# ZenHKD/ocr-vi-invoice

Measured on AMD Instinct MI355X. Metric: invoice images/sec end-to-end (det+rec), higher is better.
Workload: dtype f16x2

## Files before the change

### ocr_vi_invoice_amd/csrc/attention.hip

```cpp
#include <stdlib.h>

#include "kernels.h"

namespace ocrvi {
OCRVI_RANGE_FLAG_TU()


template <typename T> struct AttnCfg;
template <> struct AttnCfg<float> {
    static constexpr int KROW = 128;
    static constexpr __host__ __device__ int vstride(int NP) { return NP * 4 + 16; }
};
template <> struct AttnCfg<bf16_t> {
    static constexpr int KROW = 64;
    static constexpr __host__ __device__ int vstride(int NP) { return (NP * 2 + 255) / 256 * 256 + 16; }
};
template <> struct AttnCfg<f16_t> : AttnCfg<bf16_t> {};
template <> struct AttnCfg<f16x2_t> : AttnCfg<float> {};

__device__ __forceinline__ int swz64(int row) { return (-(row >> 2)) & 3; }

template <typename T> __device__ __forceinline__ f32x4 mfma16(const uint4& a, const uint4& b, f32x4 c);
template <> __device__ __forceinline__ f32x4 mfma16<bf16_t>(const uint4& a, const uint4& b, f32x4 c) {
    return __builtin_amdgcn_mfma_f32_16x16x32_bf16(__builtin_bit_cast(bf16x8, a), __builtin_bit_cast(bf16x8, b), c, 0, 0, 0);
}
template <> __device__ __forceinline__ f32x4 mfma16<f16_t>(const uint4& a, const uint4& b, f32x4 c) {
    return __builtin_amdgcn_mfma_f32_16x16x32_f16(__builtin_bit_cast(f16x8, a), __builtin_bit_cast(f16x8, b), c, 0, 0, 0);
}

__device__ __forceinline__ void split_pair(float a, float b, unsigned& H, unsigned& L) {
    typedef float f2v __attribute__((ext_vector_type(2)));
    typedef _Float16 h2v __attribute__((ext_vector_type(2)));
    H = __builtin_bit_cast(unsigned, __builtin_convertvector((f2v){a, b}, h2v));
    const float la = fma_mix_lo(-1.0f, H, a), lb = fma_mix_hi(-1.0f, H, b);
    L = __builtin_bit_cast(unsigned, __builtin_convertvector((f2v){la, lb}, h2v));
}

template <typename T, int MAXT, bool MASK, int NWV = 4>
__global__ __launch_bounds__(NWV * 64, (IsSplit<T>::value && MAXT <= 16 && NWV == 8) ? 4 : 1) void attention_kernel(const T* __restrict__ qkv, T* __restrict__ out, int N, int heads, int kbase, int Nk,
                                                                                                               float* __restrict__ po, float2* __restrict__ pml) {
    constexpr int EPC = TypeInfo<T>::EPC;
    constexpr int KROW = AttnCfg<T>::KROW;
    constexpr int CH = KROW / 16;
    extern __shared__ __attribute__((aligned(16))) char smem[];
    const int L = xcd_remap(blockIdx.x, gridDim.x);
    const int h = L % heads, b = L / heads;
    const int D = heads * 32, ld = 3 * D;
    constexpr int NP = ((MAXT + 1) / 2) * 32;
    constexpr int VS = AttnCfg<T>::vstride(NP);
    char* Ks = smem;
    char* Vt = smem + (size_t)NP * KROW;
    const int tid = threadIdx.x, lane = tid & 63, wave = tid >> 6;
    const T* base = qkv + (size_t)b * N * ld + h * 32;

    for (int idx = tid; idx < NP * CH; idx += NWV * 64) {
        const int key = idx / CH, ch = idx % CH;
        uint4 kv = make_uint4(0, 0, 0, 0), vv = make_uint4(0, 0, 0, 0);
        if (key < Nk) {
            kv = *(const uint4*)(base + (size_t)(kbase + key) * ld + D + ch * EPC);
            vv = *(const uint4*)(base + (size_t)(kbase + key) * ld + 2 * D + ch * EPC);
        }
        const int sw = sizeof(T) == 4 ? swz128(key) : swz64(key);
        if constexpr (IsSplit<T>::value) {
            char* kr = Ks + key * KROW + (ch & 1) * 8;
            *(uint2*)(kr + (((ch & ~1) ^ sw) << 4)) = make_uint2(kv.x, kv.y);
            *(uint2*)(kr + (((ch | 1) ^ sw) << 4)) = make_uint2(kv.z, kv.w);
            union { uint4 u; f16_t h[8]; } r;
            r.u = vv;
            const int vo = (key >> 5) * 128 + ((key >> 2) & 3) * 32 + (((key >> 4) & 1) * 4 + (key & 3)) * 2;
#pragma unroll
            for (int e = 0; e < 4; ++e) {
                char* dst = Vt + (ch * 4 + e) * VS + vo;
                *(f16_t*)dst = r.h[e];
                *(f16_t*)(dst + 16) = r.h[4 + e];
            }
        } else {
            *(uint4*)(Ks + key * KROW + ((ch ^ sw) << 4)) = kv;
            union { uint4 u; T e[EPC]; } r;
            r.u = vv;
#pragma unroll
            for (int e = 0; e < EPC; ++e) *(T*)(Vt + (ch * EPC + e) * VS + key * (int)sizeof(T)) = r.e[e];
        }
    }
    __syncthreads();

    const int lr = lane & 15, g = lane >> 4;
    const float c2 = 0.17677669529663687f * 1.4426950408889634f;
    const int NQ = (N + 15) >> 4;
    for (int qt = wave; qt < NQ; qt += NWV) {
        const int q = qt * 16 + lr;
        const bool qok = q < N;
        f32x4 acc[MAXT];
        int lds_off = 0;
        if (MAXT > 8) asm volatile("" : "+v"(lds_off));
        const char* Ksq = Ks + lds_off;
        const char* Vtq = Vt + lds_off;
        if constexpr (sizeof(T) == 4) {
            uint4 qf[2] = {make_uint4(0, 0, 0, 0), make_uint4(0, 0, 0, 0)};
            if (qok) {
                qf[0] = *(const uint4*)(base + (size_t)q * ld + 8 * g);
                qf[1] = *(const uint4*)(base + (size_t)q * ld + 8 * g + 4);
            }
            const int sw = swz128(lr);
            const int o0 = ((2 * g) ^ sw) << 4, o1 = ((2 * g + 1) ^ sw) << 4;
            if constexpr (IsSplit<T>::value) {
                typedef typename Mma<T>::u4v U;
                U qH, qL;
                Mma<T>::regroup(qf[0], qf[1], qH, qL);
                uint4 kq[2][2];
                auto kread = [&](int t, int set) {
                    const char* kr = Ksq + (t * 16 + lr) * KROW;
                    kq[set][0] = *(const uint4*)(kr + o0);
                    kq[set][1] = *(const uint4*)(kr + o1);
                };
                constexpr bool PRE = !(MAXT <= 16 && NWV == 8 && (MASK || MAXT == 16));
                if constexpr (PRE) {
                    kread(0, 0);
                    __builtin_amdgcn_sched_barrier(0);
                }
#pragma unroll
                for (int t = 0; t < MAXT; ++t) {
                    if constexpr (PRE) {
                        if (t + 1 < MAXT) kread(t + 1, (t + 1) & 1);
                        __builtin_amdgcn_sched_barrier(0);
                    } else {
                        kread(t, t & 1);
                    }
                    acc[t] = (f32x4){0.f, 0.f, 0.f, 0.f};
                    const uint4 k0 = kq[t & 1][0], k1 = kq[t & 1][1];
                    const U kH = {k0.x, k0.y, k0.z, k0.w}, kL = {k1.x, k1.y, k1.z, k1.w};
                    Mma<T>::three(kH, kL, qH, qL, acc[t]);
                    if constexpr (PRE) __builtin_amdgcn_sched_barrier(0);
                }
            } else {
#pragma unroll
                for (int t = 0; t < MAXT; ++t) {
                    acc[t] = (f32x4){0.f, 0.f, 0.f, 0.f};
                    const char* kr = Ksq + (t * 16 + lr) * KROW;
                    const uint4 kf0 = *(const uint4*)(kr + o0), kf1 = *(const uint4*)(kr + o1);
                    Mma<T>::half(kf0, qf[0], acc[t]);
                    Mma<T>::half(kf1, qf[1], acc[t]);
                }
            }
        } else {
            uint4 qf = make_uint4(0, 0, 0, 0);
            if (qok) qf = *(const uint4*)(base + (size_t)q * ld + 8 * g);
            const int o0 = (g ^ swz64(lr)) << 4;
#pragma unroll
            for (int t = 0; t < MAXT; ++t) {
                acc[t] = (f32x4){0.f, 0.f, 0.f, 0.f};
                acc[t] = mfma16<T>(*(const uint4*)(Ksq + (t * 16 + lr) * KROW + o0), qf, acc[t]);
            }
        }
        float mx = -INFINITY;
        if constexpr (MASK) {
            int nlim = Nk - 4 * g;
            asm volatile("" : "+v"(nlim));
#pragma unroll
            for (int t = 0; t < MAXT; ++t)
#pragma unroll
                for (int r = 0; r < 4; ++r) acc[t][r] = (t * 16 + r >= nlim) ? -INFINITY : acc[t][r];
        }
#pragma unroll
        for (int t = 0; t < MAXT; ++t)
#pragma unroll
            for (int r = 0; r < 4; ++r) mx = fmaxf(mx, acc[t][r]);
        mx = fmaxf(mx, __shfl_xor(mx, 16));
        mx = fmaxf(mx, __shfl_xor(mx, 32));
        const float nm = -mx * c2 + (IsSplit<T>::value ? 12.0f : 0.0f);
        float sum = 0.f;
        if constexpr (IsSplit<T>::value && !(MASK && MAXT == 16 && NWV == 8)) {
            typedef float f2v __attribute__((ext_vector_type(2)));
            const f2v c2v = {c2, c2}, nmv = {nm, nm};
            f2v sum2 = {0.f, 0.f};
#pragma unroll
            for (int t = 0; t < MAXT; ++t) {
#pragma unroll
                for (int h = 0; h < 2; ++h) {
                    f2v e = __builtin_elementwise_fma((f2v){acc[t][2 * h], acc[t][2 * h + 1]}, c2v, nmv);
                    e[0] = __builtin_amdgcn_exp2f(e[0]);
                    e[1] = __builtin_amdgcn_exp2f(e[1]);
                    sum2 += e;
                    acc[t][2 * h] = e[0];
                    acc[t][2 * h + 1] = e[1];
                }
            }
            sum = sum2[0] + sum2[1];
        } else {
#pragma unroll
            for (int t = 0; t < MAXT; ++t) {
#pragma unroll
                for (int r = 0; r < 4; ++r) {
                    const float p = __builtin_amdgcn_exp2f(__builtin_fmaf(acc[t][r], c2, nm));
                    acc[t][r] = p;
                    if constexpr (sizeof(T) == 4) sum += p;
                }
            }
        }
        f32x4 o[2] = {(f32x4){0.f, 0.f, 0.f, 0.f}, (f32x4){0.f, 0.f, 0.f, 0.f}};
        f32x4 osum = (f32x4){0.f, 0.f, 0.f, 0.f};
        if constexpr (IsSplit<T>::value) {
            constexpr int NS = (MAXT + 1) / 2;
            uint4 vq[2][2][2];
            auto vread = [&](int s, int set) {
#pragma unroll
                for (int dt = 0; dt < 2; ++dt) {
                    const char* vr = Vtq + (dt * 16 + lr) * VS + 128 * s + 32 * g;
                    vq[set][dt][0] = *(const uint4*)vr;
                    vq[set][dt][1] = *(const uint4*)(vr + 16);
                }
            };
            constexpr bool PRE = !(MAXT <= 16 && NWV == 8 && (MASK || MAXT == 16));
            if constexpr (PRE) {
                vread(0, 0);
                __builtin_amdgcn_sched_barrier(0);
            }
#pragma unroll
            for (int s = 0; s < NS; ++s) {
                if constexpr (PRE) {
                    if (s + 1 < NS) vread(s + 1, (s + 1) & 1);
                    __builtin_amdgcn_sched_barrier(0);
                } else {
                    vread(s, s & 1);
                }
                typedef typename Mma<T>::u4v U;
                unsigned h0, h1, h2 = 0u, h3 = 0u, l0, l1, l2 = 0u, l3 = 0u;
                split_pair(acc[2 * s][0], acc[2 * s][1], h0, l0);
                split_pair(acc[2 * s][2], acc[2 * s][3], h1, l1);
                if (2 * s + 1 < MAXT) {
                    const int t1 = 2 * s + 1 < MAXT ? 2 * s + 1 : 0;
                    split_pair(acc[t1][0], acc[t1][1], h2, l2);
                    split_pair(acc[t1][2], acc[t1][3], h3, l3);
                }
                const U pH = {h0, h1, h2, h3}, pL = {l0, l1, l2, l3};
#pragma unroll
                for (int dt = 0; dt < 2; ++dt) {
                    const uint4 v0 = vq[s & 1][dt][0], v1 = vq[s & 1][dt][1];
                    const U vH = {v0.x, v0.y, v0.z, v0.w}, vL = {v1.x, v1.y, v1.z, v1.w};
                    Mma<T>::three(vH, vL, pH, pL, o[dt]);
                }
                if constexpr (PRE) __builtin_amdgcn_sched_barrier(0);
            }
        } else if constexpr (sizeof(T) == 4) {
#pragma unroll
            for (int t = 0; t < MAXT; ++t) {
#pragma unroll
                    for (int dt = 0; dt < 2; ++dt) {
                        const float4 vf = *(const float4*)(Vtq + (dt * 16 + lr) * VS + (t * 16 + 4 * g) * 4);
                        o[dt] = __builtin_amdgcn_mfma_f32_16x16x4f32(vf.x, acc[t][0], o[dt], 0, 0, 0);
                        o[dt] = __builtin_amdgcn_mfma_f32_16x16x4f32(vf.y, acc[t][1], o[dt], 0, 0, 0);
                        o[dt] = __builtin_amdgcn_mfma_f32_16x16x4f32(vf.z, acc[t][2], o[dt], 0, 0, 0);
                        o[dt] = __builtin_amdgcn_mfma_f32_16x16x4f32(vf.w, acc[t][3], o[dt], 0, 0, 0);
                    }
                }
        } else {
            const T one = from_f32<T>(1.0f);
            union { T e[8]; uint4 u; } ones;
#pragma unroll
            for (int r = 0; r < 8; ++r) ones.e[r] = one;
#pragma unroll
            for (int s = 0; s < (MAXT + 1) / 2; ++s) {
                    union { T e[8]; uint4 u; } pf;
#pragma unroll
                    for (int r = 0; r < 4; ++r) {
                        pf.e[r] = from_f32<T>(acc[2 * s][r]);
                        pf.e[4 + r] = (2 * s + 1 < MAXT) ? from_f32<T>(acc[2 * s + 1 < MAXT ? 2 * s + 1 : 0][r]) : from_f32<T>(0.f);
                    }
                    osum = mfma16<T>(ones.u, pf.u, osum);
#pragma unroll
                    for (int dt = 0; dt < 2; ++dt) {
                        const char* vr = Vtq + (dt * 16 + lr) * VS + (32 * s + 4 * g) * 2;
                        const uint2 lo = *(const uint2*)vr, hi = *(const uint2*)(vr + 32);
                        o[dt] = mfma16<T>(make_uint4(lo.x, lo.y, hi.x, hi.y), pf.u, o[dt]);
                    }
                }
        }
        if constexpr (sizeof(T) == 4) {
            sum += __shfl_xor(sum, 16);
            sum += __shfl_xor(sum, 32);
        } else {
            sum = osum[0];
        }
        if (po) {
            if (qok) {
                float* prow = po + ((size_t)b * N + q) * D + h * 32 + 4 * g;
#pragma unroll
                for (int dt = 0; dt < 2; ++dt) *(float4*)(prow + dt * 16) = make_float4(o[dt][0], o[dt][1], o[dt][2], o[dt][3]);
                if (g == 0) pml[((size_t)b * heads + h) * N + q] = make_float2(mx, sum);
            }
            continue;
        }
        const float inv = 1.f / sum;
        if (qok) {
            T* orow = out + ((size_t)b * N + q) * D + h * 32 + 4 * g;
#pragma unroll
            for (int dt = 0; dt < 2; ++dt) {
                if constexpr (sizeof(T) == 4) {
                    const float ov[4] = {o[dt][0] * inv, o[dt][1] * inv, o[dt][2] * inv, o[dt][3] * inv};
                    store4<T>(orow + dt * 16, ov);
                } else {
                    union { T e[4]; uint2 u; } pk;
#pragma unroll
                    for (int r = 0; r < 4; ++r) pk.e[r] = from_f32<T>(o[dt][r] * inv);
                    *(uint2*)(orow + dt * 16) = pk.u;
                }
            }
        }
    }
}

typedef short short4v __attribute__((ext_vector_type(4)));

template <typename T, int NW, bool MASK>
__global__ __launch_bounds__(NW * 64) void attention16_kernel(const T* __restrict__ qkv, T* __restrict__ out, int N, int heads) {
    extern __shared__ __attribute__((aligned(16))) char smem[];
    const int L = xcd_remap(blockIdx.x, gridDim.x);
    const int h = L % heads, b = L / heads;
    const int D = heads * 32, ld = 3 * D;
    const int NB = (N + 31) >> 5;
    char* const Ks = smem;
    char* const Vs = smem + (size_t)NB * 32 * 64;
    const int tid = threadIdx.x, lane = tid & 63, wave = tid >> 6;
    const T* base = qkv + (size_t)b * N * ld + h * 32;

    for (int idx = tid; idx < NB * 32 * 8; idx += NW * 64) {
        const int key = idx >> 3, c = idx & 7;
        uint4 v = make_uint4(0, 0, 0, 0);
        if (key < N) v = *(const uint4*)(base + (size_t)key * ld + (c < 4 ? D + c * 8 : 2 * D + (c - 4) * 8));
        if (c < 4) {
            *(uint4*)(Ks + key * 64 + ((c ^ swz64(key)) << 4)) = v;
        } else {
            if ((key >> 2) & 1) v = make_uint4(v.z, v.w, v.x, v.y);
            *(uint4*)(Vs + key * 64 + ((c - 4) << 4)) = v;
        }
    }
    __syncthreads();

    const int lr = lane & 15, g = lane >> 4;
    const float c2 = 0.17677669529663687f * 1.4426950408889634f;
    const char* const kbase = Ks + lr * 64 + ((g ^ swz64(lr)) << 4);
    const int tq = (lane >> 2) & 3, tp = lane & 3;
    const unsigned vaddr0 = (unsigned)(size_t)(__attribute__((address_space(3))) char*)Vs + (4 * g + tq) * 64 + 16 * tp;
    const unsigned vsel = (g & 1) * 8;
    const T one = from_f32<T>(1.0f);
    union { T e[8]; uint4 u; } ones;
#pragma unroll
    for (int r = 0; r < 8; ++r) ones.e[r] = one;

    const int NT = (N + 31) >> 5;
    for (int task = wave; task < NT; task += NW) {
        uint4 qf[2];
#pragma unroll
        for (int qt = 0; qt < 2; ++qt) {
            const int q = task * 32 + 16 * qt + lr;
            qf[qt] = make_uint4(0, 0, 0, 0);
            if (q < N) qf[qt] = *(const uint4*)(base + (size_t)q * ld + 8 * g);
        }
        f32x4 m4[2] = {(f32x4){-INFINITY, -INFINITY, -INFINITY, -INFINITY}, (f32x4){-INFINITY, -INFINITY, -INFINITY, -INFINITY}};
        auto tile_max = [&](int t, bool mask) {
            const uint4 kf = *(const uint4*)(kbase + t * 1024);
#pragma unroll
            for (int qt = 0; qt < 2; ++qt) {
                f32x4 sc = mfma16<T>(kf, qf[qt], (f32x4){0.f, 0.f, 0.f, 0.f});
                if (mask) {
#pragma unroll
                    for (int r = 0; r < 4; ++r) sc[r] = (16 * t + 4 * g + r >= N) ? -INFINITY : sc[r];
                }
#pragma unroll
                for (int r = 0; r < 4; ++r) m4[qt][r] = fmaxf(m4[qt][r], sc[r]);
            }
        };
        const int full16 = MASK ? (N >> 4) : 2 * NB;
        for (int t = 0; t < full16; ++t) tile_max(t, false);
        if constexpr (MASK) {
            for (int t = full16; t < 2 * NB; ++t) tile_max(t, true);
        }
        float nm[2];
#pragma unroll
        for (int qt = 0; qt < 2; ++qt) {
            float mx = fmaxf(fmaxf(m4[qt][0], m4[qt][1]), fmaxf(m4[qt][2], m4[qt][3]));
            mx = fmaxf(mx, __shfl_xor(mx, 16));
            mx = fmaxf(mx, __shfl_xor(mx, 32));
            nm[qt] = -mx * c2;
        }
        f32x4 o[2][2], osum[2];
#pragma unroll
        for (int qt = 0; qt < 2; ++qt) {
            o[qt][0] = o[qt][1] = (f32x4){0.f, 0.f, 0.f, 0.f};
            osum[qt] = (f32x4){0.f, 0.f, 0.f, 0.f};
        }
        auto block = [&](int s, bool mask) {
            const uint4 kf0 = *(const uint4*)(kbase + s * 2048), kf1 = *(const uint4*)(kbase + s * 2048 + 1024);
            uint4 vf[2];
#pragma unroll
            for (int dt = 0; dt < 2; ++dt) {
                const unsigned a = vaddr0 + s * 2048 + ((8 * dt) ^ vsel);
                const short4v lo = __builtin_amdgcn_ds_read_tr16_b64_v4i16((__attribute__((address_space(3))) short4v*)(size_t)a);
                const short4v hi = __builtin_amdgcn_ds_read_tr16_b64_v4i16((__attribute__((address_space(3))) short4v*)(size_t)(a + 1024));
                union { short4v v[2]; uint4 u; } pk;
                pk.v[0] = lo; pk.v[1] = hi;
                vf[dt] = pk.u;
            }
#pragma unroll
            for (int qt = 0; qt < 2; ++qt) {
                f32x4 s0 = mfma16<T>(kf0, qf[qt], (f32x4){0.f, 0.f, 0.f, 0.f});
                f32x4 s1 = mfma16<T>(kf1, qf[qt], (f32x4){0.f, 0.f, 0.f, 0.f});
                if (mask) {
#pragma unroll
                    for (int r = 0; r < 4; ++r) {
                        s0[r] = (32 * s + 4 * g + r >= N) ? -INFINITY : s0[r];
                        s1[r] = (32 * s + 16 + 4 * g + r >= N) ? -INFINITY : s1[r];
                    }
                }
                union { T e[8]; uint4 u; } pf;
#pragma unroll
                for (int r = 0; r < 4; ++r) {
                    pf.e[r] = from_f32<T>(__builtin_amdgcn_exp2f(__builtin_fmaf(s0[r], c2, nm[qt])));
                    pf.e[4 + r] = from_f32<T>(__builtin_amdgcn_exp2f(__builtin_fmaf(s1[r], c2, nm[qt])));
                }
                osum[qt] = mfma16<T>(ones.u, pf.u, osum[qt]);
                o[qt][0] = mfma16<T>(vf[0], pf.u, o[qt][0]);
                o[qt][1] = mfma16<T>(vf[1], pf.u, o[qt][1]);
            }
        };
        const int full32 = MASK ? (N >> 5) : NB;
        for (int s = 0; s < full32; ++s) block(s, false);
        if constexpr (MASK) {
            for (int s = full32; s < NB; ++s) block(s, true);
        }
#pragma unroll
        for (int qt = 0; qt < 2; ++qt) {
            const int q = task * 32 + 16 * qt + lr;
            if (q < N) {
                const float inv = 1.f / osum[qt][0];
                union { T e[8]; uint4 u; } pk;
#pragma unroll
                for (int r = 0; r < 4; ++r) {
                    pk.e[r] = from_f32<T>(o[qt][0][r] * inv);
                    pk.e[4 + r] = from_f32<T>(o[qt][1][r] * inv);
                }
                *(uint4*)(out + ((size_t)b * N + q) * D + h * 32 + 8 * g) = pk.u;
            }
        }
    }
}

template <typename T, int NW>
static int launch_attn16(const void* qkv, void* out, int B, int N, int heads, hipStream_t s) {
    const int NB = (N + 31) / 32;
    const int smem = NB * 32 * 128;
    if (N % 32 == 0) {
        auto kern = attention16_kernel<T, NW, false>;
        OCRVI_TRY(ensure_max_smem((const void*)kern, smem));
        hipLaunchKernelGGL(kern, dim3(heads * B), dim3(NW * 64), smem, s, (const T*)qkv, (T*)out, N, heads);
    } else {
        auto kern = attention16_kernel<T, NW, true>;
        OCRVI_TRY(ensure_max_smem((const void*)kern, smem));
        hipLaunchKernelGGL(kern, dim3(heads * B), dim3(NW * 64), smem, s, (const T*)qkv, (T*)out, N, heads);
    }
    OCRVI_HIP(hipGetLastError());
    return OCRVI_OK;
}
template <typename T>
static int attn16_dt(const void* qkv, void* out, int B, int N, int heads, hipStream_t s) {
    return launch_attn16<T, 8>(qkv, out, B, N, heads, s);
}

template <typename T, int MAXT, bool MASK>
static int launch_attn_m(const void* qkv, void* out, int B, int N, int heads, hipStream_t s, int kbase, int Nk, float* po, float2* pml) {
    constexpr int NP = ((MAXT + 1) / 2) * 32;
    const int smem = NP * AttnCfg<T>::KROW + 32 * AttnCfg<T>::vstride(NP);
    if constexpr (sizeof(T) == 4 && MAXT >= 30) {
        static const bool w8 = !(getenv("OCRVI_ATTN_F32_W8") && atoi(getenv("OCRVI_ATTN_F32_W8")) == 0);
        if (w8) {
            auto kern8 = attention_kernel<T, MAXT, MASK, 8>;
            OCRVI_TRY(ensure_max_smem((const void*)kern8, smem));
            hipLaunchKernelGGL(kern8, dim3(heads * B), dim3(512), smem, s, (const T*)qkv, (T*)out, N, heads, kbase, Nk, po, pml);
            OCRVI_HIP(hipGetLastError());
            return OCRVI_OK;
        }
    }
    if constexpr (IsSplit<T>::value && MAXT >= 15 && MAXT <= 16) {
        static const bool w8 = !(getenv("OCRVI_ATTN_X2_W8") && atoi(getenv("OCRVI_ATTN_X2_W8")) == 0);
        if (w8) {
            auto kern8 = attention_kernel<T, MAXT, MASK, 8>;
            OCRVI_TRY(ensure_max_smem((const void*)kern8, smem));
            hipLaunchKernelGGL(kern8, dim3(heads * B), dim3(512), smem, s, (const T*)qkv, (T*)out, N, heads, kbase, Nk, po, pml);
            OCRVI_HIP(hipGetLastError());
            return OCRVI_OK;
        }
    }
    auto kern = attention_kernel<T, MAXT, MASK, 4>;
    OCRVI_TRY(ensure_max_smem((const void*)kern, smem));
    hipLaunchKernelGGL(kern, dim3(heads * B), dim3(256), smem, s, (const T*)qkv, (T*)out, N, heads, kbase, Nk, po, pml);
    OCRVI_HIP(hipGetLastError());
    return OCRVI_OK;
}

template <typename T, int MAXT>
static int launch_attn(const void* qkv, void* out, int B, int N, int heads, hipStream_t s, int kbase, int Nk, float* po, float2* pml) {
    if (Nk == MAXT * 16) return launch_attn_m<T, MAXT, false>(qkv, out, B, N, heads, s, kbase, Nk, po, pml);
    return launch_attn_m<T, MAXT, true>(qkv, out, B, N, heads, s, kbase, Nk, po, pml);
}

template <typename T>
static int attn_range(const void* qkv, void* out, int B, int N, int heads, hipStream_t s, int kbase, int Nk, float* po, float2* pml) {
    const int NT = (Nk + 15) >> 4;
    if (NT <= 4) return launch_attn<T, 4>(qkv, out, B, N, heads, s, kbase, Nk, po, pml);
    if (NT <= 5) return launch_attn<T, 5>(qkv, out, B, N, heads, s, kbase, Nk, po, pml);
    if (NT <= 8) return launch_attn<T, 8>(qkv, out, B, N, heads, s, kbase, Nk, po, pml);
    if (NT <= 15) return launch_attn<T, 15>(qkv, out, B, N, heads, s, kbase, Nk, po, pml);
    if (NT <= 16) return launch_attn<T, 16>(qkv, out, B, N, heads, s, kbase, Nk, po, pml);
    if (NT <= 30) return launch_attn<T, 30>(qkv, out, B, N, heads, s, kbase, Nk, po, pml);
    return launch_attn<T, 32>(qkv, out, B, N, heads, s, kbase, Nk, po, pml);
}

template <typename T>
__global__ void attention_combine_kernel(const float* __restrict__ po, const float2* __restrict__ pml, T* __restrict__ out, int B, int N, int heads, int nchunk) {
    const int D = heads * 32;
    const size_t total = (size_t)B * N * heads * 8;
    const size_t rowsD = (size_t)B * N * D, rowsH = (size_t)B * heads * N;
    const float c2 = 0.17677669529663687f * 1.4426950408889634f;
    for (size_t i = (size_t)blockIdx.x * blockDim.x + threadIdx.x; i < total; i += (size_t)gridDim.x * blockDim.x) {
        const int c4 = (int)(i & 7);
        const size_t t = i >> 3;
        const int h = (int)(t % heads);
        const size_t bq = t / heads;
        const size_t b = bq / N, q = bq % N;
        float m = -INFINITY;
        for (int c = 0; c < nchunk; ++c) m = fmaxf(m, pml[c * rowsH + (b * heads + h) * N + q].x);
        float acc[4] = {0.f, 0.f, 0.f, 0.f}, den = 0.f;
        for (int c = 0; c < nchunk; ++c) {
            const float2 ml = pml[c * rowsH + (b * heads + h) * N + q];
            const float w = __builtin_amdgcn_exp2f((ml.x - m) * c2);
            const float4 o = *(const float4*)(po + c * rowsD + bq * D + h * 32 + c4 * 4);
            acc[0] += w * o.x; acc[1] += w * o.y; acc[2] += w * o.z; acc[3] += w * o.w;
            den += w * ml.y;
        }
        const float inv = 1.f / den;
        const float ov[4] = {acc[0] * inv, acc[1] * inv, acc[2] * inv, acc[3] * inv};
        store4<T>(out + bq * D + h * 32 + c4 * 4, ov);
    }
}

static inline int attn_chunks(int N) { return (N + 511) / 512; }
static inline int attn_chunk_keys(int N) { return (int)align_up((size_t)cdiv(N, attn_chunks(N)), 32); }

template <typename T>
static int attn_dt(const void* qkv, void* out, int B, int N, int heads, hipStream_t s, void* scratch) {
    if (N <= 512) return attn_range<T>(qkv, out, B, N, heads, s, 0, N, nullptr, nullptr);
    if constexpr (sizeof(T) == 4) {
        OCRVI_CHECK(scratch, OCRVI_EINVAL, "attention: %d keys need the chunk scratch (attention_scratch_bytes)", N);
        const int nc = attn_chunks(N), ck = attn_chunk_keys(N);
        const size_t rowsD = (size_t)B * N * heads * 32, rowsH = (size_t)B * heads * N;
        float* po = (float*)scratch;
        float2* pml = (float2*)(po + (size_t)nc * rowsD);
        for (int c = 0; c < nc; ++c) {
            const int k0 = c * ck, nk = std::min(ck, N - k0);
            OCRVI_TRY(attn_range<T>(qkv, out, B, N, heads, s, k0, nk, po + (size_t)c * rowsD, pml + (size_t)c * rowsH));
        }
        const size_t total = rowsH * 8;
        hipLaunchKernelGGL(attention_combine_kernel<T>, dim3((unsigned)std::min<size_t>((total + 255) / 256, 65535)), dim3(256), 0, s, po, pml, (T*)out, B, N, heads, nc);
        OCRVI_HIP(hipGetLastError());
        return OCRVI_OK;
    } else {
        set_error("attention: the register-resident 16-bit kernel takes at most 512 keys");
        return OCRVI_EINVAL;
    }
}

size_t attention_scratch_bytes(int dtype, int B, int N, int heads) {
    if (dtype_size(dtype) != 4 || N <= 512) return 0;
    return (size_t)attn_chunks(N) * ((size_t)B * N * heads * 32 * 4 + (size_t)B * heads * N * 8);
}

int k_attention(int dtype, const void* qkv, void* out, int B, int N, int heads, hipStream_t s, void* scratch) {
    OCRVI_CHECK(qkv && out && B > 0 && B < 65536 && heads > 0 && N > 0, OCRVI_EINVAL, "attention: bad shape B=%d N=%d heads=%d", B, N, heads);
    OCRVI_CHECK(N <= (dtype_size(dtype) == 2 ? 1024 : 4096), OCRVI_EINVAL, "attention: sequence length %d unsupported (at most %d tokens in this mode)", N,
                dtype_size(dtype) == 2 ? 1024 : 4096);
    char tag[64];
    snprintf(tag, sizeof(tag), "attention_hd32_%s", dtype_name(dtype));
    const double esz = (double)dtype_size(dtype);
    ProfScope ps(tag, 4.0 * B * heads * (double)N * N * 32, (double)B * N * heads * 32 * 4 * esz, s);
    static const bool streaming = !(getenv("OCRVI_ATTN_STREAM") && atoi(getenv("OCRVI_ATTN_STREAM")) == 0);
    OCRVI_CHECK((size_t)B * heads < ((size_t)1 << 31), OCRVI_EINVAL, "attention: too many (sequence, head) pairs");
    switch (dtype) {
        case OCRVI_F32: return attn_dt<float>(qkv, out, B, N, heads, s, scratch);
        case OCRVI_BF16: return (streaming && N > 256) || N > 512 ? attn16_dt<bf16_t>(qkv, out, B, N, heads, s) : attn_dt<bf16_t>(qkv, out, B, N, heads, s, scratch);
        case OCRVI_F16: return (streaming && N > 256) || N > 512 ? attn16_dt<f16_t>(qkv, out, B, N, heads, s) : attn_dt<f16_t>(qkv, out, B, N, heads, s, scratch);
        case OCRVI_F16X2: return attn_dt<f16x2_t>(qkv, out, B, N, heads, s, scratch);
    }
    set_error("unknown dtype %d", dtype);
    return OCRVI_EINVAL;
}

}
```

Before: 323.3.

## Batch K/V staging loads and prefetch next Q tile in f16x2 attention

For the split f16x2 attention path, K/V staging now issues all global loads up front into registers, clamping indices instead of branching, and then writes them to LDS. V is transposed with packed 16-bit shuffles instead of scalar half stores. The next query tile's Q fragment is prefetched during the current tile's compute, and output stores are deferred to overlap with the next tile's work. This trades more registers for hiding global-memory latency. A compile-time cycle-profiling variant behind a build flag is also added.

```diff
diff --git a/ocr_vi_invoice_amd/csrc/attention.hip b/ocr_vi_invoice_amd/csrc/attention.hip
--- a/ocr_vi_invoice_amd/csrc/attention.hip
+++ b/ocr_vi_invoice_amd/csrc/attention.hip
@@ -36,7 +36,9 @@
     L = __builtin_bit_cast(unsigned, __builtin_convertvector((f2v){la, lb}, h2v));
 }
 
-template <typename T, int MAXT, bool MASK, int NWV = 4>
+__device__ __forceinline__ uint4 keep4(bool c, const uint4& v) { return make_uint4(c ? v.x : 0u, c ? v.y : 0u, c ? v.z : 0u, c ? v.w : 0u); }
+
+template <typename T, int MAXT, bool MASK, int NWV = 4, bool PROF = false>
 __global__ __launch_bounds__(NWV * 64, (IsSplit<T>::value && MAXT <= 16 && NWV == 8) ? 4 : 1) void attention_kernel(const T* __restrict__ qkv, T* __restrict__ out, int N, int heads, int kbase, int Nk,
                                                                                                                float* __restrict__ po, float2* __restrict__ pml) {
     constexpr int EPC = TypeInfo<T>::EPC;
@@ -52,29 +54,96 @@
     char* Vt = smem + (size_t)NP * KROW;
     const int tid = threadIdx.x, lane = tid & 63, wave = tid >> 6;
     const T* base = qkv + (size_t)b * N * ld + h * 32;
-
-    for (int idx = tid; idx < NP * CH; idx += NWV * 64) {
-        const int key = idx / CH, ch = idx % CH;
-        uint4 kv = make_uint4(0, 0, 0, 0), vv = make_uint4(0, 0, 0, 0);
-        if (key < Nk) {
-            kv = *(const uint4*)(base + (size_t)(kbase + key) * ld + D + ch * EPC);
-            vv = *(const uint4*)(base + (size_t)(kbase + key) * ld + 2 * D + ch * EPC);
-        }
-        const int sw = sizeof(T) == 4 ? swz128(key) : swz64(key);
-        if constexpr (IsSplit<T>::value) {
-            char* kr = Ks + key * KROW + (ch & 1) * 8;
-            *(uint2*)(kr + (((ch & ~1) ^ sw) << 4)) = make_uint2(kv.x, kv.y);
-            *(uint2*)(kr + (((ch | 1) ^ sw) << 4)) = make_uint2(kv.z, kv.w);
-            union { uint4 u; f16_t h[8]; } r;
-            r.u = vv;
-            const int vo = (key >> 5) * 128 + ((key >> 2) & 3) * 32 + (((key >> 4) & 1) * 4 + (key & 3)) * 2;
-#pragma unroll
-            for (int e = 0; e < 4; ++e) {
-                char* dst = Vt + (ch * 4 + e) * VS + vo;
-                *(f16_t*)dst = r.h[e];
-                *(f16_t*)(dst + 16) = r.h[4 + e];
-            }
-        } else {
+    long long tk[8] = {0, 0, 0, 0, 0, 0, 0, 0}, t0 = 0;
+    if constexpr (PROF) t0 = clock64();
+    auto tick = [&](int k) {
+        if constexpr (PROF) {
+            const long long t = clock64();
+            tk[k] += t - t0;
+            t0 = t;
+        }
+    };
+    auto tick_after = [&](int k, float last) {
+        if constexpr (PROF) {
+            asm volatile("" ::"v"(last + 1.0f));
+            tick(k);
+        }
+    };
+
+    constexpr int QA = !IsSplit<T>::value ? 0 : MAXT <= 8 ? 1 : !(NWV == 8 && MAXT <= 16) ? 2 : 0;
+    uint4 qn[2];
+    const T* qbase = base;
+    if constexpr (IsSplit<T>::value) asm volatile("" : "+s"(qbase));
+    auto qload = [&](int qt) {
+        const int qc = min(qt * 16 + (lane & 15), N - 1);
+        typedef unsigned u4n __attribute__((ext_vector_type(4)));
+        const unsigned qo = (unsigned)(qc * ld + 8 * (lane >> 4)) * 4u;
+        const __attribute__((address_space(1))) u4n* qp = (const __attribute__((address_space(1))) u4n*)((const __attribute__((address_space(1))) char*)qbase + qo);
+        const u4n q0 = qp[0], q1 = qp[1];
+        qn[0] = make_uint4(q0.x, q0.y, q0.z, q0.w);
+        qn[1] = make_uint4(q1.x, q1.y, q1.z, q1.w);
+    };
+
+    if constexpr (IsSplit<T>::value) {
+        constexpr int NTH = NWV * 64, NI = 2 * NP, NR = (NI + NTH - 1) / NTH;
+        static_assert(NI % 64 == 0, "items fill whole waves: i < NI is wave-uniform");
+        const T* kb = base + (size_t)kbase * ld + D;
+        uint4 kq[NR][4], vq[NR][4];
+#pragma unroll
+        for (int r = 0; r < NR; ++r) {
+            const int i = r * NTH + tid, l = i & 63;
+            const int kgk = i >> 3, chk = i & 7;
+            const int kgv = (i >> 6) * 8 + (l & 1) + ((l >> 4) & 1) * 2 + ((l >> 1) & 1) * 4, chv = ((l >> 2) & 3) + (l >> 5) * 4;
+#pragma unroll
+            for (int j = 0; j < 4; ++j) kq[r][j] = *(const uint4*)(kb + min(4 * kgk + j, Nk - 1) * ld + chk * EPC);
+#pragma unroll
+            for (int j = 0; j < 4; ++j) vq[r][j] = *(const uint4*)(kb + min(4 * kgv + j, Nk - 1) * ld + D + chv * EPC);
+        }
+        if constexpr (QA > 0) qload(wave);
+        __builtin_amdgcn_sched_barrier(0);
+        if constexpr (PROF) {
+            asm volatile("s_waitcnt vmcnt(0)" ::: "memory");
+            tick(0);
+        }
+#pragma unroll
+        for (int r = 0; r < NR; ++r) {
+            const int i = r * NTH + tid, l = i & 63;
+            if (NI % NTH != 0 && i >= NI) break;
+            const int kgk = i >> 3, chk = i & 7;
+            const int kgv = (i >> 6) * 8 + (l & 1) + ((l >> 4) & 1) * 2 + ((l >> 1) & 1) * 4, chv = ((l >> 2) & 3) + (l >> 5) * 4;
+#pragma unroll
+            for (int j = 0; j < 4; ++j) {
+                const int key = 4 * kgk + j, sw = swz128(key);
+                const uint4 kv = keep4(key < Nk, kq[r][j]);
+                char* kr = Ks + key * KROW + (chk & 1) * 8;
+                *(uint2*)(kr + (((chk & ~1) ^ sw) << 4)) = make_uint2(kv.x, kv.y);
+                *(uint2*)(kr + (((chk | 1) ^ sw) << 4)) = make_uint2(kv.z, kv.w);
+            }
+            uint4 vv[4];
+#pragma unroll
+            for (int j = 0; j < 4; ++j) vv[j] = keep4(4 * kgv + j < Nk, vq[r][j]);
+            const int vo = (kgv >> 3) * 128 + (kgv & 3) * 32 + ((kgv >> 2) & 1) * 8;
+            auto lo16 = [](unsigned a, unsigned b) { return (a & 0xffffu) | (b << 16); };
+            auto hi16 = [](unsigned a, unsigned b) { return (a >> 16) | (b & 0xffff0000u); };
+            char* dst = Vt + chv * 4 * VS + vo;
+            *(uint2*)(dst) = make_uint2(lo16(vv[0].x, vv[1].x), lo16(vv[2].x, vv[3].x));
+            *(uint2*)(dst + 16) = make_uint2(lo16(vv[0].z, vv[1].z), lo16(vv[2].z, vv[3].z));
+            *(uint2*)(dst + VS) = make_uint2(hi16(vv[0].x, vv[1].x), hi16(vv[2].x, vv[3].x));
+            *(uint2*)(dst + VS + 16) = make_uint2(hi16(vv[0].z, vv[1].z), hi16(vv[2].z, vv[3].z));
+            *(uint2*)(dst + 2 * VS) = make_uint2(lo16(vv[0].y, vv[1].y), lo16(vv[2].y, vv[3].y));
+            *(uint2*)(dst + 2 * VS + 16) = make_uint2(lo16(vv[0].w, vv[1].w), lo16(vv[2].w, vv[3].w));
+            *(uint2*)(dst + 3 * VS) = make_uint2(hi16(vv[0].y, vv[1].y), hi16(vv[2].y, vv[3].y));
+            *(uint2*)(dst + 3 * VS + 16) = make_uint2(hi16(vv[0].w, vv[1].w), hi16(vv[2].w, vv[3].w));
+        }
+    } else {
+        for (int idx = tid; idx < NP * CH; idx += NWV * 64) {
+            const int key = idx / CH, ch = idx % CH;
+            uint4 kv = make_uint4(0, 0, 0, 0), vv = make_uint4(0, 0, 0, 0);
+            if (key < Nk) {
+                kv = *(const uint4*)(base + (size_t)(kbase + key) * ld + D + ch * EPC);
+                vv = *(const uint4*)(base + (size_t)(kbase + key) * ld + 2 * D + ch * EPC);
+            }
+            const int sw = sizeof(T) == 4 ? swz128(key) : swz64(key);
             *(uint4*)(Ks + key * KROW + ((ch ^ sw) << 4)) = kv;
             union { uint4 u; T e[EPC]; } r;
             r.u = vv;
@@ -82,11 +151,25 @@
             for (int e = 0; e < EPC; ++e) *(T*)(Vt + (ch * EPC + e) * VS + key * (int)sizeof(T)) = r.e[e];
         }
     }
+    if constexpr (PROF) {
+        asm volatile("s_waitcnt lgkmcnt(0)" ::: "memory");
+        tick(1);
+    }
     __syncthreads();
+    if constexpr (PROF) tick(2);
 
     const int lr = lane & 15, g = lane >> 4;
     const float c2 = 0.17677669529663687f * 1.4426950408889634f;
     const int NQ = (N + 15) >> 4;
+    uint4 pend[2];
+    T* prow = out;
+    bool pok = false;
+    auto flush = [&]() {
+        if (pok) {
+            *(uint4*)prow = pend[0];
+            *(uint4*)(prow + 16) = pend[1];
+        }
+    };
     for (int qt = wave; qt < NQ; qt += NWV) {
         const int q = qt * 16 + lr;
         const bool qok = q < N;
@@ -97,7 +180,14 @@
         const char* Vtq = Vt + lds_off;
         if constexpr (sizeof(T) == 4) {
             uint4 qf[2] = {make_uint4(0, 0, 0, 0), make_uint4(0, 0, 0, 0)};
-            if (qok) {
+            if constexpr (PROF) {
+                asm volatile("s_waitcnt vmcnt(0)" ::: "memory");
+                tick(3);
+            }
+            if constexpr (QA > 0) {
+                qf[0] = keep4(qok, qn[0]);
+                qf[1] = keep4(qok, qn[1]);
+            } else if (qok) {
                 qf[0] = *(const uint4*)(base + (size_t)q * ld + 8 * g);
                 qf[1] = *(const uint4*)(base + (size_t)q * ld + 8 * g + 4);
             }
@@ -132,6 +222,13 @@
                     Mma<T>::three(kH, kL, qH, qL, acc[t]);
                     if constexpr (PRE) __builtin_amdgcn_sched_barrier(0);
                 }
+                if constexpr (PROF) tick_after(4, acc[MAXT - 1][3]);
+                if constexpr (QA == 2) {
+                    qload(qt + NWV);
+                    flush();
+                    pok = false;
+                    __builtin_amdgcn_sched_barrier(0);
+                }
             } else {
 #pragma unroll
                 for (int t = 0; t < MAXT; ++t) {
@@ -197,6 +294,7 @@
                 }
             }
         }
+        if constexpr (PROF) tick_after(5, sum);
         f32x4 o[2] = {(f32x4){0.f, 0.f, 0.f, 0.f}, (f32x4){0.f, 0.f, 0.f, 0.f}};
         f32x4 osum = (f32x4){0.f, 0.f, 0.f, 0.f};
         if constexpr (IsSplit<T>::value) {
@@ -241,6 +339,8 @@
                 }
                 if constexpr (PRE) __builtin_amdgcn_sched_barrier(0);
             }
+            if constexpr (PROF) tick_after(6, o[1][3]);
+            if constexpr (QA == 1) qload(qt + NWV);
         } else if constexpr (sizeof(T) == 4) {
 #pragma unroll
             for (int t = 0; t < MAXT; ++t) {
@@ -291,7 +391,18 @@
             continue;
         }
         const float inv = 1.f / sum;
-        if (qok) {
+        if constexpr (QA == 2) {
+            pok = qok;
+            if (qok) {
+                prow = out + ((size_t)b * N + q) * D + h * 32 + 4 * g;
+#pragma unroll
+                for (int dt = 0; dt < 2; ++dt) {
+                    const float ov[4] = {o[dt][0] * inv, o[dt][1] * inv, o[dt][2] * inv, o[dt][3] * inv};
+                    f16x2_raise(f16x2_out_of_range(ov));
+                    pend[dt] = Chunk<T>::pack(ov);
+                }
+            }
+        } else if (qok) {
             T* orow = out + ((size_t)b * N + q) * D + h * 32 + 4 * g;
 #pragma unroll
             for (int dt = 0; dt < 2; ++dt) {
@@ -306,6 +417,12 @@
                 }
             }
         }
+        if constexpr (PROF) tick(7);
+    }
+    if constexpr (QA == 2) flush();
+    if constexpr (PROF) {
+        if (lane == 0)
+            for (int k = 0; k < 8; ++k) atomicAdd((unsigned long long*)pml + k, (unsigned long long)tk[k]);
     }
 }
 
@@ -470,6 +587,29 @@
 static int launch_attn_m(const void* qkv, void* out, int B, int N, int heads, hipStream_t s, int kbase, int Nk, float* po, float2* pml) {
     constexpr int NP = ((MAXT + 1) / 2) * 32;
     const int smem = NP * AttnCfg<T>::KROW + 32 * AttnCfg<T>::vstride(NP);
+#ifdef OCRVI_RING_PROF_BUILD
+    if constexpr (IsSplit<T>::value) {
+        static const bool prof = getenv("OCRVI_RING_PROF") && atoi(getenv("OCRVI_RING_PROF"));
+        if (prof && !po) {
+            constexpr int W = MAXT >= 15 ? 8 : 4;
+            static unsigned long long* dbuf = nullptr;
+            if (!dbuf) OCRVI_HIP(hipMalloc((void**)&dbuf, 64));
+            OCRVI_HIP(hipMemsetAsync(dbuf, 0, 64, s));
+            auto kp = attention_kernel<T, MAXT, MASK, W, true>;
+            OCRVI_TRY(ensure_max_smem((const void*)kp, smem));
+            hipLaunchKernelGGL(kp, dim3(heads * B), dim3(W * 64), smem, s, (const T*)qkv, (T*)out, N, heads, kbase, Nk, (float*)nullptr, (float2*)dbuf);
+            unsigned long long hv[8];
+            OCRVI_HIP(hipMemcpyAsync(hv, dbuf, 64, hipMemcpyDeviceToHost, s));
+            OCRVI_HIP(hipStreamSynchronize(s));
+            const double w = (double)heads * B * W;
+            double tot = 0;
+            for (int k = 0; k < 8; ++k) tot += (double)hv[k];
+            fprintf(stderr, "attention f16x2 B %d N %d heads %d tiles %d mask %d waves %d: cycles/wave stage-load %.0f stage-store %.0f barrier %.0f q-wait %.0f qk %.0f softmax %.0f pv %.0f out %.0f total %.0f\n",
+                    B, N, heads, MAXT, (int)MASK, W, hv[0] / w, hv[1] / w, hv[2] / w, hv[3] / w, hv[4] / w, hv[5] / w, hv[6] / w, hv[7] / w, tot / w);
+            return OCRVI_OK;
+        }
+    }
+#endif
     if constexpr (sizeof(T) == 4 && MAXT >= 30) {
         static const bool w8 = !(getenv("OCRVI_ATTN_F32_W8") && atoi(getenv("OCRVI_ATTN_F32_W8")) == 0);
         if (w8) {
@@ -584,6 +724,7 @@
     ProfScope ps(tag, 4.0 * B * heads * (double)N * N * 32, (double)B * N * heads * 32 * 4 * esz, s);
     static const bool streaming = !(getenv("OCRVI_ATTN_STREAM") && atoi(getenv("OCRVI_ATTN_STREAM")) == 0);
     OCRVI_CHECK((size_t)B * heads < ((size_t)1 << 31), OCRVI_EINVAL, "attention: too many (sequence, head) pairs");
+    OCRVI_CHECK((size_t)N * heads * 96 * 4 < ((size_t)1 << 31), OCRVI_EINVAL, "attention: a sequence of %d tokens x %d heads is beyond 2 GB", N, heads);
     switch (dtype) {
         case OCRVI_F32: return attn_dt<float>(qkv, out, B, N, heads, s, scratch);
         case OCRVI_BF16: return (streaming && N > 256) || N > 512 ? attn16_dt<bf16_t>(qkv, out, B, N, heads, s) : attn_dt<bf16_t>(qkv, out, B, N, heads, s, scratch);
```

Result: no change. 325.4 (median of 6 runs) (+0.7%).
